# druskus20/volym

Measured on AMD Instinct MI355X. Metric: Mrays/s + achieved HBM GB/s, 256^3 uint8 @ 1920x1080, higher is better.
Workload: dtype u8 voxels, f32 compositing

## Files before the change

### volym_amd/csrc/raymarch.hip

```cpp
#include <hip/hip_runtime.h>

#include <algorithm>
#include <cmath>
#include <cstdio>
#include <chrono>
#include <cstring>
#include <queue>
#include <string>
#include <vector>

#include "context.hpp"
#include "worklist.hpp"
#include "raymarch_kernels.h"
#include "raymarch_pq.h"
#include "raymarch_pool.h"
#include "blit.h"

namespace volym {
extern template __global__ void volym_raymarch_pq_kernel<true, false, false, 4, false, false, false, PQ_WAVES, 0, false, true>(
    const uint8_t* __restrict__, const uint8_t* __restrict__, const FrameTables* __restrict__, const uint8_t* __restrict__, const uint2* __restrict__, uint32_t,
    uint16_t* __restrict__, uint32_t* __restrict__, uint32_t* __restrict__, float4* __restrict__, Counters* __restrict__, uint4* __restrict__, const FrameParams);
}

using namespace volym;
// ... 164 lines not shown
        return hull_edges(pts, 8, out);
    };
    const double c0[3] = {0, 0, 0}, c1[3] = {1, 1, 1};
    if (project_box(c0, c1, fp.hull[0])) fp.cull |= CULL_CUBE_HULL;
    if (!none && project_box(lo, hi, fp.hull[1])) {
        fp.cull |= CULL_OBJ_HULL;
        const double x0 = std::max(0.0, std::floor((bb[0] - 3.0) / PL_SBW) * PL_SBW), y0 = std::max(0.0, std::floor((bb[1] - 3.0) / PL_SBH) * PL_SBH);
        const double x1 = std::min(static_cast<double>(fp.rect[2]), std::ceil((bb[2] + 3.0) / PL_SBW) * PL_SBW), y1 = std::min(static_cast<double>(fp.rect[3]), std::ceil((bb[3] + 3.0) / PL_SBH) * PL_SBH);
        if (x1 > x0 && y1 > y0) { fp.rect[0] = static_cast<uint32_t>(x0); fp.rect[1] = static_cast<uint32_t>(y0); fp.rect[2] = static_cast<uint32_t>(x1); fp.rect[3] = static_cast<uint32_t>(y1); }
        else { fp.rect[0] = fp.rect[1] = fp.rect[2] = fp.rect[3] = 0; }
    }
    if (none) { fp.rect[0] = fp.rect[1] = fp.rect[2] = fp.rect[3] = 0; }
    fp.mask_t8x = c->tiles_x * 2u;
    s.mask_margin = static_cast<float>(margin);
    for (int i = 0; i < 16; ++i) s.mask_clip[i] = static_cast<float>(M[i]);
    s.mask_wanted = (fp.cull & CULL_OBJ_HULL) != 0u && c->tile_mask && c->tile_mask_words != 0u;
}

static void feedback_thread(const volym_ctx* c, FrameSlot* sp)
{
    FrameSlot& s = *sp;
    (void)hipSetDevice(c->device);
    for (;;) {
        {
            std::unique_lock<std::mutex> lk(s.fb_mu);
            s.fb_cv.wait(lk, [&] { const int st = s.fb_state.load(std::memory_order_acquire); return st == FrameSlot::FB_CAPTURED || st == FrameSlot::FB_QUIT; });
        }
        if (s.fb_state.load(std::memory_order_acquire) == FrameSlot::FB_QUIT) return;
        FbJob& job = s.fb_job;
        job.error.clear();
        auto now_us = [] { return std::chrono::duration<double, std::micro>(std::chrono::steady_clock::now().time_since_epoch()).count(); };
        job.t_us[1] = now_us();
        hipError_t e = hipEventSynchronize(s.ev_cost);
        job.t_us[2] = now_us();
        const int next = job.list ^ 1;
        if (e == hipSuccess) {
            const WorkList& ran = s.lists[job.list];
            const bool same_view = s.view_serial.load(std::memory_order_relaxed) == job.launch.view_serial && ran.view_serial == job.launch.view_serial;
            bool trimmed = false;
            if (same_view && ran.trimmable && ran.trim_round < job.set.trim_rounds)
                trimmed = trim_list(job.set, job.launch, s.list_capacity, ran, reinterpret_cast<const uint32_t*>(s.h_cost_pinned + ((job.n_entries + 1u) & ~1u)), s.lists[next]);
            job.t_us[3] = now_us();
            if (!trimmed) {
                costs_to_items(ran, s.h_cost_pinned, job.n_entries, s.item_cost);
                job.t_us[3] = now_us();
                const bool moving = s.view_serial.load(std::memory_order_relaxed) != job.launch.view_serial;
                deal_list(shard_grid(c), job.set, job.launch, moving, s.item_cost, s.item_is_dp, c->geometric, s.lists[next]);
            }
            job.t_us[4] = now_us();
            if (s.lists[next].entries.size() > s.list_capacity) {
                job.error = "work list larger than its buffers";
            } else {
                list_to_device_form(shard_grid(c), s.lists[next].entries, s.h_list_pinned);
                e = hipMemcpyAsync(s.d_list[next], s.h_list_pinned, s.lists[next].entries.size() * 2u * sizeof(uint32_t), hipMemcpyHostToDevice, s.copy_stream);
                if (e == hipSuccess) e = hipEventRecord(s.ev_list, s.copy_stream);
                if (e == hipSuccess) e = hipEventSynchronize(s.ev_list);
            }
        }
        if (e != hipSuccess) job.error = std::string("cost feedback: ") + hipGetErrorString(e);
        job.t_us[5] = now_us();
        {
            std::lock_guard<std::mutex> lk(s.fb_mu);
            s.fb_state.store(FrameSlot::FB_READY, std::memory_order_release);
        }
        s.fb_cv.notify_all();
    }
}

static void feedback_poll(FrameSlot& s)
{
    if (s.fb_state.load(std::memory_order_acquire) != FrameSlot::FB_READY) return;
    if (s.fb_job.error.empty()) s.cur = s.fb_job.list ^ 1;
    s.fb_state.store(FrameSlot::FB_IDLE, std::memory_order_release);
}

static void feedback_quiesce(FrameSlot& s)
{
    if (s.fb_state.load(std::memory_order_acquire) == FrameSlot::FB_CAPTURED) {
        std::unique_lock<std::mutex> lk(s.fb_mu);
        s.fb_cv.wait(lk, [&] { return s.fb_state.load(std::memory_order_acquire) != FrameSlot::FB_CAPTURED; });
    }
    feedback_poll(s);
}

int volym::quiesce_slots(volym_ctx* c)
{
    HIPCHK(c, hipSetDevice(c->device));
    for (int i = 0; i < c->n_slots(); ++i) {
        feedback_quiesce(*c->slots[i]);
        HIPCHK(c, hipStreamSynchronize(c->slots[i]->stream));
    }
    return VOLYM_OK;
}

static int reset_slot_lists(volym_ctx* c, FrameSlot& s)
{
    const size_t need = static_cast<size_t>(c->n_local) * 16u + 2u * static_cast<size_t>(c->n_cus) * 8u + 64u;
    if (need > s.list_capacity) {
        for (int i = 0; i < 2; ++i) { if (s.d_list[i]) (void)hipFree(s.d_list[i]); s.d_list[i] = nullptr; }
        if (s.d_cost) (void)hipFree(s.d_cost);
        if (s.h_list_pinned) (void)hipHostFree(s.h_list_pinned);
        if (s.h_cost_pinned) (void)hipHostFree(s.h_cost_pinned);
        s.d_cost = nullptr; s.h_list_pinned = nullptr; s.h_cost_pinned = nullptr; s.list_capacity = 0;
        hipError_t e = hipMalloc(&s.d_list[0], need * 2u * sizeof(uint32_t));
        if (e == hipSuccess) e = hipMalloc(&s.d_list[1], need * 2u * sizeof(uint32_t));
        const size_t cost_bytes = (need + 2u) * sizeof(uint16_t) + (static_cast<size_t>(c->n_cus) * 8u * (PQ_WAVES + 1u) + 64u) * sizeof(uint32_t);
// ... 527 lines not shown
}

template <bool COUNT, bool TRACE = false>
static int launch_march(volym_ctx* c, FrameSlot& s)
{
    int rc = ensure_frame_resources(c, s);
    if (rc != VOLYM_OK) return rc;
    FrameParams fp = s.fp;
    fp.rank = c->rank; fp.world = c->world; fp.n_local = c->n_local;
    fp.mc_n = c->mc_n;
    fp.xcd_bands = c->xcd_bands;
    if (c->world == 1) fp.flags |= F_RASTER;
    if (c->write_f32 && c->world == 1) fp.flags |= F_WRITE_F32;
    if (c->n_local == 0) return VOLYM_OK;
    uint32_t grid = c->n_local;
    if (fp.xcd_bands) {
        const uint32_t chunks = 8u * fp.xcd_bands;
        const uint32_t per_chunk = (c->n_local + chunks - 1u) / chunks;
        grid = per_chunk * chunks;
    }
    uint32_t* const d_shard = c->shard_buf(s);
    uint32_t* const d_frame = c->frame_buf(s);
    Counters* cnt = (COUNT || (VOLYM_DEV_SWITCHES && (s.fp.dev & 512u))) ? s.d_counters : nullptr;
    uint4* trace = TRACE ? s.d_trace : nullptr;
    if (!COUNT && !TRACE && frame_uses_pool(c, fp.flags)) {
        const uint32_t pgrid = std::min(256u, max_grid(c));
        uint32_t* dbg = s.pool_dbg ? s.d_pool_dbg : nullptr;
        if (c->bricked)
            hipLaunchKernelGGL((volym_raymarch_pool_kernel<true>), dim3(pgrid), dim3(PL_WAVES * 64), 0, s.stream, c->d_vol, s.d_tables, s.d_df, s.d_pool_sync, d_shard,
                               d_frame, s.d_f32, dbg, fp);
        else
            hipLaunchKernelGGL((volym_raymarch_pool_kernel<false>), dim3(pgrid), dim3(PL_WAVES * 64), 0, s.stream, c->d_vol, s.d_tables, s.d_df, s.d_pool_sync, d_shard,
                               d_frame, s.d_f32, dbg, fp);
        HIPCHK(c, hipGetLastError());
        s.pool_launched = true;
        return VOLYM_OK;
    }
    if (c->kernel_variant >= 2) {
        const bool plain = !COUNT && !TRACE;
        if (plain) feedback_poll(s);
        const WorkList& wl = s.lists[s.cur];
        const uint32_t n_items = static_cast<uint32_t>(wl.entries.size());
        if (n_items == 0) return VOLYM_OK;
        const bool capture = plain && c->feedback && !c->feedback_frozen && s.fb_state.load(std::memory_order_acquire) == FrameSlot::FB_IDLE && (wl.view_serial != s.view_serial.load(std::memory_order_relaxed) || !wl.final_for_view);
        uint16_t* cost_out = capture ? s.d_cost : nullptr;
        const bool table = !(fp.flags & (F_LINEAR | F_GAUSSIAN));
        const bool special = !COUNT && !(fp.flags & F_IMP_COLORING) && (fp.flags & F_OPACITY);
        const bool no_imp = special && !(fp.flags & F_IMP_RENDERING);
        const bool ir = special && (fp.flags & F_IMP_RENDERING);
        const bool wide12 = c->wide_waves == 12 || (c->wide_waves == 0 && c->bricked && ir);
        const uint32_t waves = ((table && no_imp) || !wide12) ? PQ_WAVES : PQ_WAVES_WIDE;
        const uint32_t want = (n_items + waves - 1) / waves;
        const uint32_t pgrid = wl.grid ? wl.grid : std::max(1u, std::min(want, max_grid(c)));
#define VOLYM_PQ_LAUNCH_J(T, KS, I, B, R, WV, J)                                                                                 \
    hipLaunchKernelGGL((volym_raymarch_pq_kernel<T, COUNT && I, TRACE, KS, I, B, R, WV, J>), dim3(pgrid), dim3(WV * 64), 0, s.stream, c->d_vol,  \
                       c->d_imp, s.d_tables, s.d_df, reinterpret_cast<const uint2*>(s.d_list[s.cur]), n_items, cost_out, d_shard, d_frame, s.d_f32, cnt, trace, fp)
#define VOLYM_PQ_LAUNCH(T, KS, I, B, R, WV) VOLYM_PQ_LAUNCH_J(T, KS, I, B, R, WV, 0)
#if VOLYM_DEV_SWITCHES
#define VOLYM_PQ_LAUNCH_W(T, KS, I, B, R) do { if (wide12) VOLYM_PQ_LAUNCH(T, KS, I, B, R, PQ_WAVES_WIDE); else VOLYM_PQ_LAUNCH(T, KS, I, B, R, PQ_WAVES); } while (0)
#else
#define VOLYM_PQ_LAUNCH_W(T, KS, I, B, R) VOLYM_PQ_LAUNCH(T, KS, I, B, R, PQ_WAVES)
#endif
        const bool cone_jobs = ir && (fp.flags & F_CONE) != 0u && !TRACE;
        const bool straight_jobs = VOLYM_DEV_SWITCHES && ir && !(fp.flags & F_CONE) && !TRACE && c->straight_jobs;
        (void)straight_jobs;
        if (c->bricked) {
#if VOLYM_DEV_SWITCHES
            if (table && no_imp && c->lds_bricks && !COUNT && !TRACE)
                hipLaunchKernelGGL((volym_raymarch_pq_kernel<true, false, false, 4, false, true, false, PQ_WAVES, 0, true>), dim3(pgrid), dim3(PQ_WAVES * 64), 0, s.stream, c->d_vol,
                                   c->d_imp, s.d_tables, s.d_df, reinterpret_cast<const uint2*>(s.d_list[s.cur]), n_items, cost_out, d_shard, d_frame, s.d_f32, cnt, trace, fp);
            else
#endif
            if (table && no_imp) VOLYM_PQ_LAUNCH(true, 4, false, true, false, PQ_WAVES);
            else if (table && ir && cone_jobs) VOLYM_PQ_LAUNCH_J(true, 4, false, true, true, PQ_WAVES, 1);
#if VOLYM_DEV_SWITCHES
            else if (table && ir && straight_jobs) VOLYM_PQ_LAUNCH_J(true, 4, false, true, true, PQ_WAVES, 2);
#endif
            else if (table && ir) { if (wide12) VOLYM_PQ_LAUNCH(true, 4, false, true, true, PQ_WAVES_WIDE); else VOLYM_PQ_LAUNCH(true, 4, false, true, true, PQ_WAVES); }
            else if (table) VOLYM_PQ_LAUNCH_W(true, 4, true, true, false);
            else VOLYM_PQ_LAUNCH_W(false, 1, true, true, false);
        } else {
            if (table && no_imp) VOLYM_PQ_LAUNCH(true, 4, false, false, false, PQ_WAVES);
            else if (table && ir && cone_jobs) VOLYM_PQ_LAUNCH_J(true, 4, false, false, true, PQ_WAVES, 1);
#if VOLYM_DEV_SWITCHES
            else if (table && ir && straight_jobs) VOLYM_PQ_LAUNCH_J(true, 4, false, false, true, PQ_WAVES, 2);
#endif
            else if (table && ir) VOLYM_PQ_LAUNCH_W(true, 4, false, false, true);
            else if (table) VOLYM_PQ_LAUNCH_W(true, 4, true, false, false);
            else VOLYM_PQ_LAUNCH_W(false, 1, true, false, false);
        }
#undef VOLYM_PQ_LAUNCH_W
#undef VOLYM_PQ_LAUNCH
#undef VOLYM_PQ_LAUNCH_J
        HIPCHK(c, hipGetLastError());
        if (capture) {
            HIPCHK(c, hipEventRecord(s.ev_march, s.stream));
            HIPCHK(c, hipStreamWaitEvent(s.copy_stream, s.ev_march, 0));
            const size_t cost_bytes = static_cast<size_t>((n_items + 1u) & ~1u) * sizeof(uint16_t) + static_cast<size_t>(pgrid) * (waves + 1u) * sizeof(uint32_t);
            HIPCHK(c, hipMemcpyAsync(s.h_cost_pinned, s.d_cost, cost_bytes, hipMemcpyDeviceToHost, s.copy_stream));
            HIPCHK(c, hipEventRecord(s.ev_cost, s.copy_stream));
            FbJob& job = s.fb_job;
            job.list = s.cur;
            job.n_entries = n_items;
            job.launch.view_serial = s.view_serial.load(std::memory_order_relaxed);
            job.launch.captured_has_dp = wl.has_dp;
            job.launch.continuous = (fp.flags & (F_LINEAR | F_GAUSSIAN)) != 0u;
// ... 530 lines not shown
```

### volym_amd/csrc/raymarch_device.h

```cpp
#pragma once

#include <hip/hip_runtime.h>

#include "wgsl_math.h"

namespace volym {

enum : uint32_t {
    F_CONE = 1u << 0,
    F_IMP_COLORING = 1u << 1,
    F_OPACITY = 1u << 2,
    F_IMP_RENDERING = 1u << 3,
    F_GAUSSIAN = 1u << 4,
    F_LINEAR = 1u << 5,
    F_WRITE_F32 = 1u << 6,
    F_RASTER = 1u << 7,
};

struct FrameParams {
    float ivp[16];
    float eye[3];
    float thr;
    float base_step;
    float min_step;
    float alpha_y;
    uint32_t flags;
    uint32_t ahead_steps;
    uint32_t W, H;
    uint32_t nx, ny, nz;
    uint32_t tiles_x, n_tiles;
    uint32_t rank, world, n_local;
    uint32_t thr_byte;
    uint32_t tf_n;
    uint32_t mc_n;
    uint32_t xcd_bands;
    float gauss_w[5];
    float cone_cos[8], cone_sin[8];
    uint32_t cull;
    float hull[2][8][4];
    float aabb_lo[3], aabb_hi[3];
    float imp_lo[3], imp_hi[3];
    uint32_t dev;
    uint32_t mask_t8x;
    const uint32_t* tile_mask;
    uint32_t* tile_mask_spare;
    uint32_t mask_words;
    const uint32_t* tile_depth;
    float rcp_w, rcp_h;
    float setup_lo;
    uint32_t rect[4];
};

template <size_t OFFSET>
__device__ __forceinline__ const FrameParams& frame_params_here()
{
    typedef const __attribute__((address_space(4))) char* kernarg_ptr;
    kernarg_ptr p = (kernarg_ptr)__builtin_amdgcn_kernarg_segment_ptr() + OFFSET;
    asm volatile("; frame_params_here: kernarg offset %1" : "+s"(p) : "n"(OFFSET));
    return *(const FrameParams*)(const char*)p;
}

#ifndef VOLYM_DEV_SWITCHES
#define VOLYM_DEV_SWITCHES 0
#endif
#define VOLYM_DF_IN_LDS(fp) (!VOLYM_DEV_SWITCHES || (fp).mc_n <= 32u)
#define VOLYM_DF_LDS_BYTES 16384

enum : uint32_t {
    CULL_CUBE_HULL = 1u << 0,
    CULL_OBJ_HULL = 1u << 1,
    CULL_AABB = 1u << 2,
    CULL_NOTHING_DENSE = 1u << 3,
    CULL_TILE_MASK = 1u << 4,
    CULL_TILE_DEPTH = 1u << 5,
};

struct FrameTables {
    float4 tf_tab[256];
    float4 lut_f[256];
    float ic_alpha[256];
    float rho[256];
};

struct Counters {
    unsigned long long n_vol, n_imp, n_steps, n_dense, n_hit;
};

struct V3 {
    float x, y, z;
};
__device__ __forceinline__ V3 v3(float x, float y, float z) { return V3{x, y, z}; }
__device__ __forceinline__ V3 operator+(V3 a, V3 b) { return v3(a.x + b.x, a.y + b.y, a.z + b.z); }
__device__ __forceinline__ V3 operator-(V3 a, V3 b) { return v3(a.x - b.x, a.y - b.y, a.z - b.z); }
__device__ __forceinline__ V3 operator*(V3 a, float s) { return v3(a.x * s, a.y * s, a.z * s); }
__device__ __forceinline__ V3 operator/(V3 a, float s) { return v3(a.x / s, a.y / s, a.z / s); }
__device__ __forceinline__ float dot_exact(V3 a, V3 b) { return (a.x * b.x + a.y * b.y) + a.z * b.z; }
__device__ __forceinline__ V3 cross(V3 a, V3 b)
{
    return v3(a.y * b.z - a.z * b.y, a.z * b.x - a.x * b.z, a.x * b.y - a.y * b.x);
}
__device__ __forceinline__ float length_exact(V3 a) { return __builtin_sqrtf(dot_exact(a, a)); }
__device__ __forceinline__ V3 normalize_exact(V3 a) { return a / length_exact(a); }
__device__ __forceinline__ float dot_fast(V3 a, V3 b)
// ... 581 lines not shown
```

### volym_amd/csrc/raymarch_pq.h

```cpp
#pragma once

#include <cstddef>
#include <type_traits>

#include "raymarch_device.h"
#include "worklist_entry.h"

namespace volym {

constexpr int PQ_WAVES = 16;
constexpr int PQ_WAVES_WIDE = 12;
constexpr uint32_t PQ_MIN_LEAP_D = 2;
constexpr int PQ_DP_DEPTH = 2;
constexpr int PQ_ITEMS_LDS = 512;
constexpr int pq_qcap(int k) { return 64 + 64 * k; }
constexpr float PQ_FIX_SCALE = 268435456.0f;
constexpr float PQ_FIX_INV = 1.0f / 268435456.0f;

__device__ __forceinline__ uint32_t lane_rank_in_mask(unsigned long long mask)
{
    return __builtin_amdgcn_mbcnt_hi(static_cast<uint32_t>(mask >> 32), __builtin_amdgcn_mbcnt_lo(static_cast<uint32_t>(mask), 0u));
}

typedef float f32x2 __attribute__((ext_vector_type(2)));

enum : uint32_t { TILE_MARCH = 0, TILE_HIT_TEST = 1, TILE_FILL_EMPTY = 2, TILE_FILL_MISS = 3 };

struct HullEdge { float a, b, c; bool valid; };
__device__ __forceinline__ HullEdge load_hull_edge(const FrameParams& fp, uint32_t lane)
{
    const uint32_t h = lane >> 5, e = (lane >> 2) & 7u;
    HullEdge r;
    r.a = fp.hull[h][e][0]; r.b = fp.hull[h][e][1]; r.c = fp.hull[h][e][2]; r.valid = fp.hull[h][e][3] > 0.5f;
    return r;
}
__device__ __forceinline__ uint32_t classify_tile(const FrameParams& fp, const HullEdge& edge, uint32_t lane, float x0, float y0, float extent = 7.0f,
                                                   bool masked_out = false)
{
    const uint32_t k = lane & 3u;
    const float cx = (k & 1u) ? x0 + extent : x0, cy = (k & 2u) ? y0 + extent : y0;
    const float a = edge.a, b = edge.b, c = edge.c;
    const bool valid = edge.valid;
    const float v = __builtin_fmaf(a, cx, __builtin_fmaf(b, cy, c));
    const float margin = 1.5f;
    const unsigned long long mo = __ballot(valid && v < -margin);
    const unsigned long long mi = __ballot(!valid || v > margin);
    auto outside = [&](uint32_t bits) { return ((bits & (bits >> 1) & (bits >> 2) & (bits >> 3)) & 0x11111111u) != 0u; };
    const bool cube_ok = (fp.cull & CULL_CUBE_HULL) != 0u, obj_ok = (fp.cull & CULL_OBJ_HULL) != 0u;
    const bool out_cube = cube_ok && outside(static_cast<uint32_t>(mo));
    const bool in_cube = cube_ok && static_cast<uint32_t>(mi) == 0xffffffffu;
    const bool out_obj = masked_out || (fp.cull & CULL_NOTHING_DENSE) != 0u || (obj_ok && outside(static_cast<uint32_t>(mo >> 32)));
    if (out_cube) return TILE_FILL_MISS;
    if (out_obj) return in_cube ? TILE_FILL_EMPTY : TILE_HIT_TEST;
    return TILE_MARCH;
}
__device__ __forceinline__ bool tile_mask_bit(const FrameParams& fp, uint32_t t8x, uint32_t t8y)
{
    const uint32_t bit = t8y * fp.mask_t8x + t8x;
    return ((fp.tile_mask[bit >> 5] >> (bit & 31u)) & 1u) != 0u;
}
struct PqKernelArgs {
    const uint8_t* vol; const uint8_t* imp; const FrameTables* tables; const uint8_t* df4; const uint2* order; uint32_t n_items; uint16_t* cost;
    uint32_t* out_shard; uint32_t* out_raster; float4* out_f32; Counters* counters; uint4* trace; FrameParams fp;
};
constexpr size_t PQ_FP_KERNARG_OFFSET = offsetof(PqKernelArgs, fp);
static_assert(PQ_FP_KERNARG_OFFSET % 8 == 0 && alignof(FrameParams) == 8, "FrameParams holds pointers: 8-byte aligned in the segment");

template <bool TABLE, bool COUNT, bool TRACE = false, int KSPEC = 1, bool IMP = true, bool BRICK = false, bool IR = false, int WAVES = PQ_WAVES, int CJ = 0, bool LB = false,
          bool RELOAD = true>
__global__ __launch_bounds__(WAVES * 64) void volym_raymarch_pq_kernel(
    const uint8_t* __restrict__ vol, const uint8_t* __restrict__ imp, const FrameTables* __restrict__ tables,
    const uint8_t* __restrict__ df4, const uint2* __restrict__ order, uint32_t n_items, uint16_t* __restrict__ cost,
    uint32_t* __restrict__ out_shard, uint32_t* __restrict__ out_raster, float4* __restrict__ out_f32,
    Counters* __restrict__ counters, uint4* __restrict__ trace, const FrameParams fp)
{
    constexpr int K = TABLE ? KSPEC : 2;
    constexpr int PQ_QCAP = pq_qcap(K);
    static_assert(K <= 4, "the shading queue of K > 4 does not fit the LDS");
    static_assert(CJ == 0 || IR, "look-ahead jobs belong to the importance-rendering instantiation");
    unsigned long long trace_t0 = 0;
    uint32_t trace_iters = 0, trace_flushes = 0, trace_tiles = 0, trace_marched = 0, trace_lanes = 0, trace_accepted = 0, trace_dp_iters = 0;
    unsigned long long tm_leap = 0, tm_samp = 0, tm_flush = 0, tm_mark = 0;
#define PQ_TICK() (TRACE ? __builtin_amdgcn_s_memtime() : 0ull)
    if (TRACE) trace_t0 = __builtin_amdgcn_s_memrealtime();

    __shared__ float4 s_tf_tab[256];
    __shared__ float4 s_lut[TABLE ? 1 : 256];
    __shared__ float s_ic_alpha[256];
    __shared__ float s_rho[256];
    __shared__ __attribute__((aligned(16))) uint8_t s_df[VOLYM_DF_LDS_BYTES];
    constexpr int THREADS = WAVES * 64;
    __shared__ float4 s_q[WAVES][PQ_QCAP];
    __shared__ uint32_t s_qm[WAVES][PQ_QCAP];
    __shared__ float s_qr[TABLE ? 1 : WAVES][TABLE ? 1 : PQ_QCAP];
    __shared__ uint32_t s_acc[WAVES][3][64];
    __shared__ float4 s_hh[WAVES][64];
    __shared__ uint8_t s_mail[(IMP || IR) ? WAVES : 1][(IMP || IR) ? 256 : 1];
    uint8_t (*const s_cres)[(IMP || IR) ? 256 : 1] = s_mail;
    constexpr uint32_t CJ_LPR = CJ == 2 ? 1u : 8u;
    constexpr uint32_t CJ_RPS = 64u / CJ_LPR;
    constexpr uint32_t CJ_CAP = CJ == 2 ? 64u : 32u;
    static_assert(!LB || (TABLE && BRICK && !IMP && !IR && !COUNT && K == 4), "LDS brick staging: bricked layout, common instantiation");
    constexpr uint32_t LB_SLOTS = 8u;
    __shared__ uint32_t s_lb[LB ? WAVES : 1][LB ? LB_SLOTS * 16u : 1u];
    constexpr int ITEMS_LDS = LB ? PQ_ITEMS_LDS / 4 : CJ == 2 ? PQ_ITEMS_LDS / 2 : PQ_ITEMS_LDS;
    __shared__ float4 s_cj[CJ ? 2 * CJ_CAP : 1];
    __shared__ uint32_t s_cj_flag[CJ ? CJ_CAP : 1];
    __shared__ uint32_t s_cj_ctl[4];
    __shared__ uint32_t s_next_ticket;
    __shared__ uint2 s_items[ITEMS_LDS];

    static_assert(!(IMP && IR), "IR specialises the IMP = false paths");
    const uint32_t flags = IMP ? fp.flags : IR ? ((fp.flags & ~F_IMP_COLORING) | F_OPACITY | F_IMP_RENDERING)
                                               : ((fp.flags & ~(F_IMP_COLORING | F_IMP_RENDERING | F_CONE)) | F_OPACITY);
    const bool linear = (flags & F_LINEAR) != 0u;
    const bool gauss = (flags & F_GAUSSIAN) != 0u;
    const bool imp_coloring = IMP && (flags & F_IMP_COLORING) != 0u;
    const bool imp_rendering = (IMP || IR) && (flags & F_IMP_RENDERING) != 0u;
    const bool need_imp = imp_coloring || imp_rendering;

    if (fp.tile_mask_spare)
        for (uint32_t wrd = blockIdx.x * (WAVES * 64u) + threadIdx.x; wrd < fp.mask_words; wrd += gridDim.x * (WAVES * 64u)) fp.tile_mask_spare[wrd] = 0u;
    if (VOLYM_DEV_SWITCHES && (fp.dev & 16u)) return;
    uint32_t* const wg_time = reinterpret_cast<uint32_t*>(cost + ((n_items + 1u) & ~1u));
    if (cost && threadIdx.x == 0u) wg_time[gridDim.x * WAVES + blockIdx.x] = static_cast<uint32_t>(__builtin_amdgcn_s_memrealtime());
    {
        const uint32_t i = threadIdx.x;
        if (i == 0u) s_next_ticket = 0u;
        if (CJ) {
            for (uint32_t k = i; k < CJ_CAP; k += THREADS) s_cj_flag[k] = 0u;
            if (i == 0u) { s_cj_ctl[0] = 0u; s_cj_ctl[1] = 0u; s_cj_ctl[2] = WAVES; }
        }
        for (uint32_t k = i; k < static_cast<uint32_t>(ITEMS_LDS); k += THREADS) {
            const size_t gi = blockIdx.x + static_cast<size_t>(gridDim.x) * k;
            if (gi < n_items) s_items[k] = order[gi];
        }
        if (i < 256u) {
            s_tf_tab[i] = tables->tf_tab[i];
            s_rho[i] = tables->rho[i];
            s_ic_alpha[i] = tables->ic_alpha[i];
            if (!TABLE) s_lut[i] = tables->lut_f[i];
        }
        {
            const uint32_t n16 = VOLYM_DF_IN_LDS(fp) ? (fp.mc_n * fp.mc_n * fp.mc_n / 2u + 15u) / 16u : 0u;
            const uint4* src = reinterpret_cast<const uint4*>(df4);
            uint4* dst = reinterpret_cast<uint4*>(s_df);
            if (!(VOLYM_DEV_SWITCHES && (fp.dev & 8u)))
                for (uint32_t k = i; k < n16; k += THREADS) dst[k] = src[k];
        }
    }
    __syncthreads();
    if (VOLYM_DEV_SWITCHES && (fp.dev & 4u)) return;

    const uint32_t lane = threadIdx.x & 63u;
    const uint32_t wave = __builtin_amdgcn_readfirstlane(threadIdx.x >> 6);

    GridT<BRICK> g;
    grid_init(g, vol, imp, fp.nx, fp.ny, fp.nz);

    float4* const q4 = s_q[wave];
    uint32_t* const qm = s_qm[wave];
    float* const qr = s_qr[TABLE ? 0 : wave];
// ... 152 lines not shown
                    const uint32_t hd = *reinterpret_cast<volatile uint32_t*>(&s_cj_ctl[0]);
                    tl = *reinterpret_cast<volatile uint32_t*>(&s_cj_ctl[1]);
                    const uint32_t room = CJ_CAP - min(CJ_CAP, tl - hd);
                    got = min(n, room);
                    if (got != 0u && atomicCAS(&s_cj_ctl[1], tl, tl + got) != tl) got = 0;
                }
                got = __builtin_amdgcn_readfirstlane(got);
                cj_count += got;
                const uint32_t first_pos = __builtin_amdgcn_readfirstlane(tl);
                if (got != 0u) {
                    const uint32_t rank = lane_rank_in_mask(m);
                    if (mine && rank < got) {
                        float tk = tsk[0];
#pragma unroll
                        for (int q = 1; q < NK; ++q) tk = k == static_cast<uint32_t>(q) ? tsk[q] : tk;
                        const V3 start = org + dir * tk;
                        const uint32_t idx = (first_pos + rank) & (CJ_CAP - 1u);
                        const float step = (t_exit - length_exact(start)) / static_cast<float>(static_cast<int>(fa.ahead_steps));
                        bool written = false;
                        uint32_t spins = 0;
                        while (!written) {
                            if (atomicCAS(&s_cj_flag[idx], 0u, 2u) == 0u) {
                                s_cj[2u * idx] = make_float4(start.x, start.y, start.z, step);
                                s_cj[2u * idx + 1u] = make_float4(dir.x, dir.y, dir.z, __uint_as_float(wave | (k << 4) | (lane << 6)));
                                __builtin_amdgcn_fence(__ATOMIC_SEQ_CST, "wavefront");
                                *reinterpret_cast<volatile uint32_t*>(&s_cj_flag[idx]) = 1u;
                                written = true;
                            } else {
                                __builtin_amdgcn_s_sleep(1);
                                if (++spins >= (1u << 20)) {
                                    *reinterpret_cast<volatile uint8_t*>(&s_cres[wave][k * 64 + lane]) = 1;
                                    written = true;
                                    if (VOLYM_DEV_SWITCHES && (fp.dev & 512u)) atomicAdd(&counters->n_dense, 1ull);
                                }
                            }
                        }
                        todo_bits &= ~(1u << k);
                        if (VOLYM_DEV_SWITCHES && (fp.dev & 512u)) atomicAdd(&counters->n_vol, 1ull);
                    }
                    if (got == n) { k++; continue; }
                }
            } else {
                bool pending = false;
#pragma unroll
                for (int q = 0; q < NK; ++q) pending = pending || (((need_bits >> q) & 1u) != 0u && *reinterpret_cast<volatile uint8_t*>(&s_cres[wave][q * 64 + lane]) == 0);
                if (__ballot(pending) == 0ull) break;
            }
            if (!cj_serve()) __builtin_amdgcn_s_sleep(1);
            if (VOLYM_DEV_SWITCHES && (fp.dev & 512u) && turns + 1u == (1u << 16) && lane == 0u) atomicAdd(&counters->n_steps, 1ull);
        }
#pragma unroll
        for (int q = 0; q < NK; ++q) found[q] = ((need_bits >> q) & 1u) != 0u && *reinterpret_cast<volatile uint8_t*>(&s_cres[wave][q * 64 + lane]) == 2;
    };
    for (uint32_t ticket = grab(); ticket < n_mine; ticket = grab()) {
      const FrameParams& fe = RELOAD ? frame_params_here<PQ_FP_KERNARG_OFFSET>() : fp;
      {
        const size_t list_pos = blockIdx.x + static_cast<size_t>(gridDim.x) * ticket;
        const uint2 entry = ticket < static_cast<uint32_t>(ITEMS_LDS) ? s_items[ticket] : order[list_pos];
        const uint32_t raw_p = __builtin_amdgcn_readfirstlane(entry.x);
        if (raw_p == PQ_NO_ITEM) continue;
        const uint32_t entry_xy = __builtin_amdgcn_readfirstlane(entry.y);
        const uint32_t tx = entry_xy & 0xffffu, ty = entry_xy >> 16;
        uint32_t entry_cost = 0;
        switch (wl_prio(raw_p)) {
            case 0: __builtin_amdgcn_s_setprio(0); break;
            case 1: __builtin_amdgcn_s_setprio(1); break;
            case 2: __builtin_amdgcn_s_setprio(2); break;
            default: __builtin_amdgcn_s_setprio(3); break;
        }
        const uint32_t raw0 = wl_code(raw_p);
        const bool is_super = wl_is_super(raw0);
        uint32_t n_sub = 1;
        if (is_super) {
            const uint32_t lt = wl_super_tile(raw0);
            const uint32_t tx16 = tx, ty16 = ty;
            bool masked16 = false;
            if (culling && (fe.cull & CULL_TILE_MASK))
                masked16 = !(tile_mask_bit(fe, tx16 * 2u, ty16 * 2u) || tile_mask_bit(fe, tx16 * 2u + 1u, ty16 * 2u) ||
                             tile_mask_bit(fe, tx16 * 2u, ty16 * 2u + 1u) || tile_mask_bit(fe, tx16 * 2u + 1u, ty16 * 2u + 1u));
            const uint32_t cls = culling ? classify_tile(fe, hull_edge, lane, static_cast<float>(tx16 * 16u), static_cast<float>(ty16 * 16u), 15.0f, masked16) : TILE_MARCH;
            if (cls >= TILE_FILL_EMPTY) {
                const uint32_t packed = cls == TILE_FILL_MISS ? 0xff000000u : 0u;
                if (flags & F_RASTER) {
                    const uint32_t gx4 = tx16 * 16u + (lane & 3u) * 4u, gy4 = ty16 * 16u + (lane >> 2);
                    if (gy4 < fe.H && (fe.W & 3u) == 0u && (reinterpret_cast<uintptr_t>(out_raster) & 15u) == 0u && gx4 < fe.W && !(flags & F_WRITE_F32)) {
                        *reinterpret_cast<uint4*>(out_raster + static_cast<size_t>(gy4) * fe.W + gx4) = make_uint4(packed, packed, packed, packed);
                    } else if (gy4 < fe.H) {
                        for (uint32_t i = 0; i < 4u; ++i)
                            if (gx4 + i < fe.W) {
                                out_raster[static_cast<size_t>(gy4) * fe.W + gx4 + i] = packed;
                                if (flags & F_WRITE_F32) out_f32[static_cast<size_t>(gy4) * fe.W + gx4 + i] = make_float4(0.0f, 0.0f, 0.0f, cls == TILE_FILL_MISS ? 1.0f : 0.0f);
                            }
                    }
                } else {
                    for (uint32_t i = 0; i < 4u; ++i) {
                        const uint32_t sl = lane * 4u + i, sub4 = sl >> 6, in = sl & 63u;
                        const uint32_t gxx = tx16 * 16u + ((sub4 & 1u) << 3) + (in & 7u), gyy = ty16 * 16u + ((sub4 >> 1) << 3) + (in >> 3);
                        out_shard[static_cast<size_t>(lt) * 256u + sl] = (gxx < fe.W && gyy < fe.H) ? packed : 0u;
                    }
                }
                if (cost && lane == 0) cost[list_pos] = 0;
                continue;
            }
            n_sub = 4;
        }
      for (uint32_t sub_iter = 0; sub_iter < n_sub; ++sub_iter) {
        const uint32_t raw = is_super ? (wl_super_tile(raw0) * 4u + sub_iter) : raw0;
        const bool is_quarter = wl_is_quarter(raw);
        const bool dp = is_quarter && !COUNT;
        const uint32_t item = is_quarter ? wl_quarter_item(raw) : raw;
        const uint32_t quarter = wl_quarter_index(raw);
        if (is_quarter && !dp && quarter != 0u) continue;
        const uint32_t local_tile = item >> 2, sub = item & 3u;
        const uint32_t px_in_sub = dp ? (((quarter & 1u) << 2) + ((lane >> 2) & 3u)) : (lane & 7u);
        const uint32_t py_in_sub = dp ? (((quarter >> 1) << 2) + (lane >> 4)) : (lane >> 3);
        const uint32_t sub_lane = py_in_sub * 8u + px_in_sub;
        const uint32_t own = dp ? (lane & ~3u) : lane;
        const uint32_t gx = tx * 16u + ((sub & 1u) << 3) + px_in_sub;
        const uint32_t gy = ty * 16u + ((sub >> 1) << 3) + py_in_sub;
        const bool in_frame = gx < fe.W && gy < fe.H;

        if (TRACE) { trace_tiles++; tm_mark = PQ_TICK(); }
        uint32_t tile_iters = 0, tile_flushes = 0, tile_trips = 0;
        const uint32_t cj_at_start = cj_count, la_at_start = la_rounds;
        uint32_t trace_ray_iters = 0;
        uint32_t tclass = TILE_MARCH;
        if (culling && !dp) {
            const bool masked8 = (fe.cull & CULL_TILE_MASK) != 0u && !tile_mask_bit(fe, tx * 2u + (sub & 1u), ty * 2u + (sub >> 1));
            tclass = classify_tile(fe, hull_edge, lane, static_cast<float>(tx * 16u + ((sub & 1u) << 3)), static_cast<float>(ty * 16u + ((sub >> 1) << 3)), 7.0f, masked8);
            if (tclass >= TILE_FILL_EMPTY) {
                const uint32_t packed = tclass == TILE_FILL_MISS ? 0xff000000u : 0u;
                if (flags & F_RASTER) {
                    if (in_frame) {
                        const size_t o = static_cast<size_t>(gy) * fe.W + gx;
                        out_raster[o] = packed;
                        if (flags & F_WRITE_F32) out_f32[o] = make_float4(0.0f, 0.0f, 0.0f, tclass == TILE_FILL_MISS ? 1.0f : 0.0f);
                    }
                } else {
                    out_shard[static_cast<size_t>(local_tile) * 256u + sub * 64u + sub_lane] = in_frame ? packed : 0u;
                }
                continue;
            }
        }
        if (TRACE) trace_marched++;

        acc_r[lane] = 0u; acc_g[lane] = 0u; acc_b[lane] = 0u;
        uint32_t q_head = 0, q_count = 0;

        Ray ray;
        ray.o = v3(0.0f, 0.0f, 0.0f); ray.d = v3(0.0f, 0.0f, 0.0f); ray.t_entry = 0.0f; ray.t_exit = 0.0f;
        ray.hit = false;
        if (in_frame) ray = make_ray<TABLE && !IMP && !IR>(fe, gx, gy);
        {
            const V3 hvec = ray_half_vector(ray.d);
            hh[lane] = make_float4(hvec.x, hvec.y, hvec.z, 0.0f);
        }
        bool active = in_frame && ray.hit;
        if (COUNT && active) n_hit++;
        float t = active ? ray.t_entry : 0.0f, cur = base, acc_a = active ? 0.0f : 1.0f;
        bool last_dense = false;
        if (culling && tclass == TILE_HIT_TEST) active = false;
        float t_end = ray.t_exit;
        if (culling && (fe.cull & CULL_AABB) && active) {
            const float rx = __builtin_amdgcn_rcpf(ray.d.x), ry = __builtin_amdgcn_rcpf(ray.d.y), rz = __builtin_amdgcn_rcpf(ray.d.z);
            const float ax0 = (fe.aabb_lo[0] - ray.o.x) * rx, ax1 = (fe.aabb_hi[0] - ray.o.x) * rx;
            const float ay0 = (fe.aabb_lo[1] - ray.o.y) * ry, ay1 = (fe.aabb_hi[1] - ray.o.y) * ry;
            const float az0 = (fe.aabb_lo[2] - ray.o.z) * rz, az1 = (fe.aabb_hi[2] - ray.o.z) * rz;
            float tn = __builtin_fmaxf(__builtin_fmaxf(__builtin_fminf(ax0, ax1), __builtin_fminf(ay0, ay1)), __builtin_fminf(az0, az1));
            float tf = __builtin_fminf(__builtin_fminf(__builtin_fmaxf(ax0, ax1), __builtin_fmaxf(ay0, ay1)), __builtin_fmaxf(az0, az1));
            tn = tn - 2.0e-5f * __builtin_fabsf(tn) - 1.0e-6f;
            tf = tf + 2.0e-5f * __builtin_fabsf(tf) + 1.0e-6f;
            if (fe.cull & CULL_TILE_DEPTH) {
                const auto* td = (const __attribute__((address_space(4))) uint32_t*)fe.tile_depth;
                const uint32_t t8 = (ty * 2u + (sub >> 1)) * fe.mask_t8x + tx * 2u + (sub & 1u);
                tn = __builtin_fmaxf(tn, __uint_as_float(~td[t8]));
                tf = __builtin_fminf(tf, __uint_as_float(td[32u * fe.mask_words + t8]));
            }
            const bool outside_static = (ray.d.x == 0.0f && (ray.o.x < fe.aabb_lo[0] || ray.o.x > fe.aabb_hi[0])) ||
                                        (ray.d.y == 0.0f && (ray.o.y < fe.aabb_lo[1] || ray.o.y > fe.aabb_hi[1])) ||
                                        (ray.d.z == 0.0f && (ray.o.z < fe.aabb_lo[2] || ray.o.z > fe.aabb_hi[2]));
            if (outside_static || !(tn <= tf)) {
// ... 678 lines not shown
```

### volym_amd/csrc/worklist.cpp

```cpp
#include "worklist.hpp"

#include <algorithm>
#include <cstdio>
#include <cstdlib>
#include <utility>

#include "../../include/volym_hip.h"

#ifndef VOLYM_DEV_SWITCHES
#define VOLYM_DEV_SWITCHES 0
#endif

using namespace volym;

static_assert(wl_code(wl_with_prio(wl_item(0x0fffffffu), 3u)) == 0x0fffffffu && wl_prio(wl_with_prio(wl_item(0x0fffffffu), 3u)) == 3u, "whole item");
static_assert(wl_is_quarter(wl_quarter(0x03ffffffu, 3u)) && !wl_is_super(wl_quarter(0x03ffffffu, 3u)) && wl_quarter_item(wl_quarter(0x03ffffffu, 3u)) == 0x03ffffffu &&
              wl_quarter_index(wl_quarter(0x03ffffffu, 3u)) == 3u && wl_local_tile(wl_quarter(0x03ffffffu, 3u)) == 0x00ffffffu, "quarter");
static_assert(wl_is_super(wl_super(0x00ffffffu)) && !wl_is_quarter(wl_super(0x00ffffffu)) && wl_super_tile(wl_super(0x00ffffffu)) == 0x00ffffffu &&
              wl_local_tile(wl_code(wl_with_prio(wl_super(0x00ffffffu), 3u))) == 0x00ffffffu, "super fill");
static_assert(!wl_is_quarter(wl_item(0u)) && !wl_is_super(wl_item(0u)) && wl_local_tile(wl_item(7u)) == 1u, "item");

std::vector<uint32_t> volym::build_geometric(const ShardGrid& g)
{
    std::vector<std::pair<uint32_t, uint32_t>> keyed;
// ... 204 lines not shown
    out.shares.assign(static_cast<size_t>(G) * rows_out, 0);
    for (uint32_t b = 0; b < G; ++b)
        for (size_t r = 0; r < wg[b].size(); ++r) {
            out.entries[r * G + b] = wg[b][r].code;
            out.shares[r * G + b] = static_cast<uint16_t>(wg[b][r].w - 1u);
        }
    out.grid = G;
    out.view_serial = in.view_serial;
    out.has_dp = in.has_dp;
    out.trimmable = true;
    out.trim_round = in.trim_round + 1;
    out.final_for_view = out.trim_round >= set.trim_rounds;
    return true;
}

void volym::list_to_device_form(const ShardGrid& g, const std::vector<uint32_t>& entries, uint32_t* out)
{
    for (size_t i = 0; i < entries.size(); ++i) {
        const uint32_t raw_p = entries[i];
        uint32_t xy = 0;
        if (raw_p != PQ_NO_ITEM) {
            const uint32_t tile = wl_local_tile(wl_code(raw_p)) * g.world + g.rank;
            xy = (tile % g.tiles_x) | ((tile / g.tiles_x) << 16);
        }
        out[2 * i] = raw_p;
        out[2 * i + 1] = xy;
    }
}

void volym::costs_to_items(const WorkList& list, const uint16_t* cost, uint32_t n_entries, std::vector<uint16_t>& item_cost)
{
    std::vector<uint32_t> q_max(item_cost.size(), 0);
    std::vector<uint8_t> q_seen(item_cost.size(), 0);
    for (uint32_t p = 0; p < n_entries && p < list.entries.size(); ++p) {
        const uint32_t raw_p = list.entries[p];
        if (raw_p == PQ_NO_ITEM) continue;
        const uint32_t raw = wl_code(raw_p);
        const uint32_t k = cost[p];
        if (wl_is_quarter(raw)) {
            const uint32_t item = wl_quarter_item(raw);
            if (item < item_cost.size()) { q_max[item] = std::max(q_max[item], k); q_seen[item] = 1; }
        } else if (wl_is_super(raw)) {
            const uint32_t lt = wl_super_tile(raw);
            for (uint32_t sub = 0; sub < 4; ++sub)
                if (lt * 4u + sub < item_cost.size()) item_cost[lt * 4u + sub] = static_cast<uint16_t>(k == 0 ? 0u : std::max(1u, k / 4u));
        } else if (raw < item_cost.size()) {
            item_cost[raw] = static_cast<uint16_t>(k);
        }
    }
    for (size_t i = 0; i < item_cost.size(); ++i)
        if (q_seen[i]) item_cost[i] = static_cast<uint16_t>(std::min(65535u, 5u + q_max[i]));
}

static WorkList list_in(const volym_wl_list& l)
{
    WorkList w;
    w.entries.assign(l.entries, l.entries + l.n);
    w.shares.assign(l.shares, l.shares + l.n);
    w.grid = l.grid; w.trim_round = l.trim_round; w.view_serial = l.view_serial;
    w.has_dp = l.has_dp != 0; w.trimmable = l.trimmable != 0; w.final_for_view = l.final_for_view != 0;
    return w;
}

static int list_out(const WorkList& w, volym_wl_list* l)
{
    if (w.entries.size() > l->capacity || w.shares.size() != w.entries.size()) return VOLYM_E_INVALID;
    std::copy(w.entries.begin(), w.entries.end(), l->entries);
    std::copy(w.shares.begin(), w.shares.end(), l->shares);
    l->n = static_cast<uint32_t>(w.entries.size());
    l->grid = w.grid; l->trim_round = w.trim_round; l->view_serial = w.view_serial;
    l->has_dp = w.has_dp; l->trimmable = w.trimmable; l->final_for_view = w.final_for_view;
    return VOLYM_OK;
}

static bool arrays(const volym_wl_list* l) { return l && l->entries && l->shares; }

extern "C" {

int volym_wl_build_geometric(const ShardGrid* g, uint32_t* out, uint32_t capacity, uint32_t* n_out)
{
    if (!g || !out || !n_out) return VOLYM_E_INVALID;
    const std::vector<uint32_t> v = build_geometric(*g);
    if (v.size() > capacity) return VOLYM_E_INVALID;
    std::copy(v.begin(), v.end(), out);
    *n_out = static_cast<uint32_t>(v.size());
    return VOLYM_OK;
}

int volym_wl_deal_list(const ShardGrid* g, const ListSettings* set, const CapturedLaunch* job, int moving, const uint16_t* cost, uint8_t* item_is_dp, uint32_t n_items,
                       const uint32_t* geometric, uint32_t n_geometric, volym_wl_list* out)
{
    if (!g || !set || !job || !cost || !item_is_dp || !geometric || !arrays(out)) return VOLYM_E_INVALID;
    std::vector<uint8_t> is_dp(item_is_dp, item_is_dp + n_items);
    WorkList w;
    deal_list(*g, *set, *job, moving != 0, std::vector<uint16_t>(cost, cost + n_items), is_dp, std::vector<uint32_t>(geometric, geometric + n_geometric), w);
    std::copy(is_dp.begin(), is_dp.end(), item_is_dp);
    return list_out(w, out);
}

int volym_wl_trim_list(const ListSettings* set, const CapturedLaunch* job, uint32_t capacity, const volym_wl_list* in, const uint32_t* times, volym_wl_list* out)
{
    if (!set || !job || !arrays(in) || !times || !arrays(out)) return VOLYM_E_INVALID;
    WorkList w;
    if (!trim_list(*set, *job, capacity, list_in(*in), times, w)) return 0;
    const int rc = list_out(w, out);
    return rc == VOLYM_OK ? 1 : rc;
}

int volym_wl_list_to_device_form(const ShardGrid* g, const uint32_t* entries, uint32_t n, uint32_t* out)
{
    if (!g || !entries || !out) return VOLYM_E_INVALID;
    list_to_device_form(*g, std::vector<uint32_t>(entries, entries + n), out);
    return VOLYM_OK;
}

int volym_wl_costs_to_items(const volym_wl_list* list, const uint16_t* cost, uint32_t n_entries, uint16_t* item_cost, uint32_t n_items)
{
    if (!arrays(list) || !cost || !item_cost) return VOLYM_E_INVALID;
    std::vector<uint16_t> v(item_cost, item_cost + n_items);
    costs_to_items(list_in(*list), cost, n_entries, v);
    std::copy(v.begin(), v.end(), item_cost);
    return VOLYM_OK;
}

}
```

### volym_amd/csrc/worklist.hpp

```cpp
#pragma once

#include <cstddef>
#include <cstdint>
#include <vector>

#include "worklist_entry.h"

namespace volym {

struct WorkList {
    std::vector<uint32_t> entries;
    uint32_t grid = 0;
    uint64_t view_serial = 0;
    bool has_dp = false;
    bool trimmable = false;
    uint32_t trim_round = 0;
    bool final_for_view = false;
    std::vector<uint16_t> shares;
};

struct ShardGrid {
    uint32_t W = 0, H = 0, tiles_x = 0, tiles_y = 0;
    uint32_t rank = 0, world = 1, n_local = 0;
};

struct ListSettings {
    int dp_min_cost = -1;
    uint32_t dp_share_pct = 60;
    uint32_t dp_floor = 64;
    int dilate = -1;
    bool super_fill = true;
    bool only_quarters = false;
    uint32_t dev_drop_tenths = 0;
    uint32_t trim_rounds = 0;
    uint32_t prio_tenths[3] = {3, 6, 10};
};

struct CapturedLaunch {
    uint64_t view_serial = 0;
    bool captured_has_dp = false;
    bool continuous = false;
    bool plain = false;
    uint32_t max_grid = 0, waves = 16;
    uint32_t grid = 0;
};

std::vector<uint32_t> build_geometric(const ShardGrid& g);
void deal_list(const ShardGrid& g, const ListSettings& set, const CapturedLaunch& job, bool moving, const std::vector<uint16_t>& measured_cost,
               std::vector<uint8_t>& item_is_dp, const std::vector<uint32_t>& geometric, WorkList& out);
bool trim_list(const ListSettings& set, const CapturedLaunch& job, size_t capacity, const WorkList& in, const uint32_t* times, WorkList& out);
void list_to_device_form(const ShardGrid& g, const std::vector<uint32_t>& entries, uint32_t* out);
void costs_to_items(const WorkList& list, const uint16_t* cost, uint32_t n_entries, std::vector<uint16_t>& item_cost);

}

extern "C" {
struct volym_wl_list {
    uint32_t* entries;
    uint16_t* shares;
    uint32_t capacity, n, grid, trim_round;
    uint64_t view_serial;
    uint8_t has_dp, trimmable, final_for_view;
};
int volym_wl_build_geometric(const volym::ShardGrid* g, uint32_t* out, uint32_t capacity, uint32_t* n_out);
int volym_wl_deal_list(const volym::ShardGrid* g, const volym::ListSettings* set, const volym::CapturedLaunch* job, int moving, const uint16_t* cost, uint8_t* item_is_dp,
                       uint32_t n_items, const uint32_t* geometric, uint32_t n_geometric, volym_wl_list* out);
int volym_wl_trim_list(const volym::ListSettings* set, const volym::CapturedLaunch* job, uint32_t capacity, const volym_wl_list* in, const uint32_t* times, volym_wl_list* out);
int volym_wl_list_to_device_form(const volym::ShardGrid* g, const uint32_t* entries, uint32_t n, uint32_t* out);
int volym_wl_costs_to_items(const volym_wl_list* list, const uint16_t* cost, uint32_t n_entries, uint16_t* item_cost, uint32_t n_items);
}
```

Measured before the change: 88590.

## Batch-classify tail work items per wave and fill empty tiles without marching

Adds a host-computed tail_row marking where the list's trailing low-cost items begin. Past that row each wave grabs a batch of up to 64 tickets at once and classifies every tile cooperatively. Empty or missed tiles are filled directly, and only tiles that still need marching are queued in a per-wave LDS bitmask. The change also reads the 16x16 tile-mask bits in one call through the constant address space, reuses them for the 8x8 subtiles, and only reclassifies when the hull test says march. The aim is to cut per-item grab and launch overhead for the many cheap, culled tail tiles, at the cost of extra wave-level serial loops and more complex ticket bookkeeping.

```diff
diff --git a/volym_amd/csrc/raymarch.hip b/volym_amd/csrc/raymarch.hip
--- a/volym_amd/csrc/raymarch.hip
+++ b/volym_amd/csrc/raymarch.hip
@@ -240,6 +240,8 @@
                 job.error = "work list larger than its buffers";
             } else {
                 list_to_device_form(shard_grid(c), s.lists[next].entries, s.h_list_pinned);
+                s.lists[next].tail_row = list_tail_row(s.lists[next].entries.data(), s.lists[next].shares.size() == s.lists[next].entries.size() ? s.lists[next].shares.data() : nullptr,
+                                                       s.lists[next].entries.size(), s.lists[next].grid);
                 e = hipMemcpyAsync(s.d_list[next], s.h_list_pinned, s.lists[next].entries.size() * 2u * sizeof(uint32_t), hipMemcpyHostToDevice, s.copy_stream);
                 if (e == hipSuccess) e = hipEventRecord(s.ev_list, s.copy_stream);
                 if (e == hipSuccess) e = hipEventSynchronize(s.ev_list);
@@ -873,6 +875,7 @@
         const uint32_t waves = ((table && no_imp) || !wide12) ? PQ_WAVES : PQ_WAVES_WIDE;
         const uint32_t want = (n_items + waves - 1) / waves;
         const uint32_t pgrid = wl.grid ? wl.grid : std::max(1u, std::min(want, max_grid(c)));
+        fp.tail_row = wl.grid ? wl.tail_row : (n_items + pgrid - 1u) / pgrid;
 #define VOLYM_PQ_LAUNCH_J(T, KS, I, B, R, WV, J)                                                                                 \
     hipLaunchKernelGGL((volym_raymarch_pq_kernel<T, COUNT && I, TRACE, KS, I, B, R, WV, J>), dim3(pgrid), dim3(WV * 64), 0, s.stream, c->d_vol,  \
                        c->d_imp, s.d_tables, s.d_df, reinterpret_cast<const uint2*>(s.d_list[s.cur]), n_items, cost_out, d_shard, d_frame, s.d_f32, cnt, trace, fp)
diff --git a/volym_amd/csrc/raymarch_device.h b/volym_amd/csrc/raymarch_device.h
--- a/volym_amd/csrc/raymarch_device.h
+++ b/volym_amd/csrc/raymarch_device.h
@@ -49,6 +49,7 @@
     float rcp_w, rcp_h;
     float setup_lo;
     uint32_t rect[4];
+    uint32_t tail_row;
 };
 
 template <size_t OFFSET>
diff --git a/volym_amd/csrc/raymarch_pq.h b/volym_amd/csrc/raymarch_pq.h
--- a/volym_amd/csrc/raymarch_pq.h
+++ b/volym_amd/csrc/raymarch_pq.h
@@ -56,8 +56,23 @@
 }
 __device__ __forceinline__ bool tile_mask_bit(const FrameParams& fp, uint32_t t8x, uint32_t t8y)
 {
+    const auto* tm = (const __attribute__((address_space(4))) uint32_t*)fp.tile_mask;
     const uint32_t bit = t8y * fp.mask_t8x + t8x;
-    return ((fp.tile_mask[bit >> 5] >> (bit & 31u)) & 1u) != 0u;
+    return ((tm[bit >> 5] >> (bit & 31u)) & 1u) != 0u;
+}
+__device__ __forceinline__ uint32_t tile_mask_bits16(const FrameParams& fp, uint32_t tx16, uint32_t ty16)
+{
+    const auto* tm = (const __attribute__((address_space(4))) uint32_t*)fp.tile_mask;
+    const uint32_t b0 = ty16 * 2u * fp.mask_t8x + tx16 * 2u, b1 = b0 + 1u, b2 = b0 + fp.mask_t8x, b3 = b2 + 1u;
+    const uint32_t w0 = tm[b0 >> 5], w1 = tm[b1 >> 5], w2 = tm[b2 >> 5], w3 = tm[b3 >> 5];
+    return ((w0 >> (b0 & 31u)) & 1u) | (((w1 >> (b1 & 31u)) & 1u) << 1) | (((w2 >> (b2 & 31u)) & 1u) << 2) | (((w3 >> (b3 & 31u)) & 1u) << 3);
+}
+__device__ __forceinline__ uint32_t classify_tile_masked(const FrameParams& fp, const HullEdge& edge, uint32_t lane, uint32_t tx16, uint32_t ty16, uint32_t want,
+                                                          float x0, float y0, float extent)
+{
+    const uint32_t cls = classify_tile(fp, edge, lane, x0, y0, extent, false);
+    if (cls != TILE_MARCH || !(fp.cull & CULL_TILE_MASK) || (tile_mask_bits16(fp, tx16, ty16) & want) != 0u) return cls;
+    return classify_tile(fp, edge, lane, x0, y0, extent, true);
 }
 struct PqKernelArgs {
     const uint8_t* vol; const uint8_t* imp; const FrameTables* tables; const uint8_t* df4; const uint2* order; uint32_t n_items; uint16_t* cost;
@@ -108,6 +123,7 @@
     __shared__ uint32_t s_cj_flag[CJ ? CJ_CAP : 1];
     __shared__ uint32_t s_cj_ctl[4];
     __shared__ uint32_t s_next_ticket;
+    __shared__ uint32_t s_tb[WAVES][4];
     __shared__ uint2 s_items[ITEMS_LDS];
 
     static_assert(!(IMP && IR), "IR specialises the IMP = false paths");
@@ -366,7 +382,64 @@
 #pragma unroll
         for (int q = 0; q < NK; ++q) found[q] = ((need_bits >> q) & 1u) != 0u && *reinterpret_cast<volatile uint8_t*>(&s_cres[wave][q * 64 + lane]) == 2;
     };
-    for (uint32_t ticket = grab(); ticket < n_mine; ticket = grab()) {
+    constexpr uint32_t TAIL_BATCH = 64u, TAIL_MIN_RUN = 4u;
+    bool tb_more = false;
+    volatile uint32_t* const tb = s_tb[wave];
+    for (;;) {
+      uint32_t ticket;
+      if (tb_more) {
+        const unsigned long long pend = static_cast<unsigned long long>(__builtin_amdgcn_readfirstlane(tb[0])) | (static_cast<unsigned long long>(__builtin_amdgcn_readfirstlane(tb[1])) << 32);
+        const uint32_t rest = __builtin_amdgcn_readfirstlane(tb[2]);
+        const uint32_t l = static_cast<uint32_t>(__builtin_ctzll(pend));
+        const unsigned long long left = pend & (pend - 1ull);
+        if (lane == 0u) { tb[0] = static_cast<uint32_t>(left); tb[1] = static_cast<uint32_t>(left >> 32); }
+        tb_more = left != 0ull;
+        ticket = rest + l - 1u;
+      } else {
+        const FrameParams& fb = fp_here();
+        const uint32_t tail_row = fb.tail_row;
+        ticket = grab();
+        if (ticket >= n_mine) break;
+        const uint32_t run = min(TAIL_BATCH, (n_mine - tail_row + static_cast<uint32_t>(WAVES) - 1u) / static_cast<uint32_t>(WAVES));
+        if (culling && ticket >= tail_row && run >= ((VOLYM_DEV_SWITCHES && (fp.dev & 1024u)) ? 1u : TAIL_MIN_RUN) && !(VOLYM_DEV_SWITCHES && (fp.dev & 64u))) {
+            uint32_t rest = 0;
+            if (run > 1u && lane == 0) rest = atomicAdd(&s_next_ticket, run - 1u);
+            rest = __builtin_amdgcn_readfirstlane(rest);
+            const uint32_t my_ticket = lane == 0u ? ticket : rest + lane - 1u;
+            const bool mine = lane < run && my_ticket < n_mine;
+            const size_t my_pos = blockIdx.x + static_cast<size_t>(gridDim.x) * my_ticket;
+            uint2 entry = make_uint2(PQ_NO_ITEM, 0u);
+            if (mine) entry = my_ticket < static_cast<uint32_t>(ITEMS_LDS) ? s_items[my_ticket] : order[my_pos];
+            const bool listed = mine && entry.x != PQ_NO_ITEM;
+            const bool plain_raster = (flags & F_RASTER) != 0u && !(flags & F_WRITE_F32);
+            const bool rows16 = (fb.W & 3u) == 0u && (reinterpret_cast<uintptr_t>(out_raster) & 15u) == 0u;
+            unsigned long long pending = 0ull;
+            for (unsigned long long todo = __ballot(listed); todo != 0ull; todo &= todo - 1ull) {
+                const int l = __builtin_ctzll(todo);
+                const uint32_t code = wl_code(static_cast<uint32_t>(__builtin_amdgcn_readlane(static_cast<int>(entry.x), l)));
+                const uint32_t exy = static_cast<uint32_t>(__builtin_amdgcn_readlane(static_cast<int>(entry.y), l));
+                const bool sup = wl_is_super(code);
+                const uint32_t sub = code & 3u;
+                const uint32_t x0 = (exy & 0xffffu) * 16u + (sup ? 0u : (sub & 1u) << 3), y0 = (exy >> 16) * 16u + (sup ? 0u : (sub >> 1) << 3);
+                uint32_t cls = TILE_MARCH;
+                if (plain_raster && (sup ? rows16 : !wl_is_quarter(code)))
+                    cls = classify_tile_masked(fb, hull_edge, lane, exy & 0xffffu, exy >> 16, sup ? 0xfu : 1u << sub, static_cast<float>(x0), static_cast<float>(y0), sup ? 15.0f : 7.0f);
+                if (cls < TILE_FILL_EMPTY) { pending |= 1ull << l; continue; }
+                const uint32_t packed = cls == TILE_FILL_MISS ? 0xff000000u : 0u;
+                if (sup) {
+                    const uint32_t gx4 = x0 + (lane & 3u) * 4u, gy4 = y0 + (lane >> 2);
+                    if (gy4 < fb.H && gx4 < fb.W) *reinterpret_cast<uint4*>(out_raster + static_cast<size_t>(gy4) * fb.W + gx4) = make_uint4(packed, packed, packed, packed);
+                } else {
+                    const uint32_t gx = x0 + (lane & 7u), gy = y0 + (lane >> 3);
+                    if (gx < fb.W && gy < fb.H) out_raster[static_cast<size_t>(gy) * fb.W + gx] = packed;
+                }
+            }
+            if (cost && listed && !((pending >> lane) & 1ull)) cost[my_pos] = 0;
+            tb_more = (pending & ~1ull) != 0ull;
+            if (tb_more && lane == 0u) { tb[0] = static_cast<uint32_t>(pending & ~1ull); tb[1] = static_cast<uint32_t>(pending >> 32); tb[2] = rest; }
+            if (!(pending & 1ull)) continue;
+        }
+      }
       const FrameParams& fe = RELOAD ? frame_params_here<PQ_FP_KERNARG_OFFSET>() : fp;
       {
         const size_t list_pos = blockIdx.x + static_cast<size_t>(gridDim.x) * ticket;
@@ -385,14 +458,16 @@
         const uint32_t raw0 = wl_code(raw_p);
         const bool is_super = wl_is_super(raw0);
         uint32_t n_sub = 1;
+        uint32_t mask16 = 0xfu;
+        if (VOLYM_DEV_SWITCHES && (fp.dev & 32u) && is_super) continue;
         if (is_super) {
             const uint32_t lt = wl_super_tile(raw0);
             const uint32_t tx16 = tx, ty16 = ty;
-            bool masked16 = false;
-            if (culling && (fe.cull & CULL_TILE_MASK))
-                masked16 = !(tile_mask_bit(fe, tx16 * 2u, ty16 * 2u) || tile_mask_bit(fe, tx16 * 2u + 1u, ty16 * 2u) ||
-                             tile_mask_bit(fe, tx16 * 2u, ty16 * 2u + 1u) || tile_mask_bit(fe, tx16 * 2u + 1u, ty16 * 2u + 1u));
-            const uint32_t cls = culling ? classify_tile(fe, hull_edge, lane, static_cast<float>(tx16 * 16u), static_cast<float>(ty16 * 16u), 15.0f, masked16) : TILE_MARCH;
+            uint32_t cls = culling ? classify_tile(fe, hull_edge, lane, static_cast<float>(tx16 * 16u), static_cast<float>(ty16 * 16u), 15.0f, false) : TILE_MARCH;
+            if (culling && cls == TILE_MARCH && (fe.cull & CULL_TILE_MASK)) {
+                mask16 = tile_mask_bits16(fe, tx16, ty16);
+                if (mask16 == 0u) cls = classify_tile(fe, hull_edge, lane, static_cast<float>(tx16 * 16u), static_cast<float>(ty16 * 16u), 15.0f, true);
+            }
             if (cls >= TILE_FILL_EMPTY) {
                 const uint32_t packed = cls == TILE_FILL_MISS ? 0xff000000u : 0u;
                 if (flags & F_RASTER) {
@@ -440,7 +515,7 @@
         uint32_t trace_ray_iters = 0;
         uint32_t tclass = TILE_MARCH;
         if (culling && !dp) {
-            const bool masked8 = (fe.cull & CULL_TILE_MASK) != 0u && !tile_mask_bit(fe, tx * 2u + (sub & 1u), ty * 2u + (sub >> 1));
+            const bool masked8 = (fe.cull & CULL_TILE_MASK) != 0u && !(is_super ? ((mask16 >> sub) & 1u) != 0u : tile_mask_bit(fe, tx * 2u + (sub & 1u), ty * 2u + (sub >> 1)));
             tclass = classify_tile(fe, hull_edge, lane, static_cast<float>(tx * 16u + ((sub & 1u) << 3)), static_cast<float>(ty * 16u + ((sub >> 1) << 3)), 7.0f, masked8);
             if (tclass >= TILE_FILL_EMPTY) {
                 const uint32_t packed = tclass == TILE_FILL_MISS ? 0xff000000u : 0u;
diff --git a/volym_amd/csrc/worklist.cpp b/volym_amd/csrc/worklist.cpp
--- a/volym_amd/csrc/worklist.cpp
+++ b/volym_amd/csrc/worklist.cpp
@@ -280,6 +280,16 @@
         if (q_seen[i]) item_cost[i] = static_cast<uint16_t>(std::min(65535u, 5u + q_max[i]));
 }
 
+uint32_t volym::list_tail_row(const uint32_t* entries, const uint16_t* shares, size_t n, uint32_t grid)
+{
+    const size_t G = std::max(1u, grid);
+    const size_t rows = (n + G - 1) / G;
+    if (!shares) return static_cast<uint32_t>(rows);
+    size_t i = n;
+    while (i > 0 && (shares[i - 1] == 0 || entries[i - 1] == PQ_NO_ITEM)) --i;
+    return static_cast<uint32_t>((i + G - 1) / G);
+}
+
 static WorkList list_in(const volym_wl_list& l)
 {
     WorkList w;
@@ -351,4 +361,11 @@
     return VOLYM_OK;
 }
 
-}
+int volym_wl_tail_row(const uint32_t* entries, const uint16_t* shares, uint32_t n, uint32_t grid, uint32_t* row_out)
+{
+    if ((!entries && n) || !row_out || grid == 0) return VOLYM_E_INVALID;
+    *row_out = list_tail_row(entries, shares, n, grid);
+    return VOLYM_OK;
+}
+
+}
diff --git a/volym_amd/csrc/worklist.hpp b/volym_amd/csrc/worklist.hpp
--- a/volym_amd/csrc/worklist.hpp
+++ b/volym_amd/csrc/worklist.hpp
@@ -17,6 +17,7 @@
     uint32_t trim_round = 0;
     bool final_for_view = false;
     std::vector<uint16_t> shares;
+    uint32_t tail_row = 0;
 };
 
 struct ShardGrid {
@@ -51,6 +52,7 @@
 bool trim_list(const ListSettings& set, const CapturedLaunch& job, size_t capacity, const WorkList& in, const uint32_t* times, WorkList& out);
 void list_to_device_form(const ShardGrid& g, const std::vector<uint32_t>& entries, uint32_t* out);
 void costs_to_items(const WorkList& list, const uint16_t* cost, uint32_t n_entries, std::vector<uint16_t>& item_cost);
+uint32_t list_tail_row(const uint32_t* entries, const uint16_t* shares, size_t n, uint32_t grid);
 
 }
 
@@ -68,4 +70,5 @@
 int volym_wl_trim_list(const volym::ListSettings* set, const volym::CapturedLaunch* job, uint32_t capacity, const volym_wl_list* in, const uint32_t* times, volym_wl_list* out);
 int volym_wl_list_to_device_form(const volym::ShardGrid* g, const uint32_t* entries, uint32_t n, uint32_t* out);
 int volym_wl_costs_to_items(const volym_wl_list* list, const uint16_t* cost, uint32_t n_entries, uint16_t* item_cost, uint32_t n_items);
+int volym_wl_tail_row(const uint32_t* entries, const uint16_t* shares, uint32_t n, uint32_t grid, uint32_t* row_out);
 }
```

New measurement: 87150. -1.6%, worse.
